# facebookresearch/Pearl

Hardware: NVIDIA H100
Metric: learner gradient-steps/sec (batch=256, 1e6 replay) (higher is better)
Workload: dtype f32 (3xTF32 tensor-core products, fp32 accumulate)

## Files before the change

### pearl_b200/csrc/dqn_tc.cu

```cuda
#include <math.h>
#include <stdarg.h>
#include <stdlib.h>

#include <new>

#include "dqn_common.cuh"
#include "sampler.cuh"
#include "umma.cuh"

using namespace prl;

int prl_sampler_params(const prl_buf *b, int k, prl::SamplerParams *sp, size_t *smem_bytes);

namespace {

constexpr int NTH = 256;
constexpr int HID = 64;
constexpr int MAX_B = 256;
constexpr int REG1 = 0, REG2 = 65536, REG3 = 131072, MISC_OFF = 196608;
constexpr int HALF = 32768;
constexpr int SBUF = 16384;
constexpr int TL = 144;
constexpr int AR_A_HI = 0, AR_A_LO = 18432, AR_E = 36864, AR_B_LO = 46080, AR_B_HI = REG3 + HALF;
constexpr int ACH = 1024, ARING = 8, ASLOT = 4 * ACH * 4;

struct TcLearner {
    const uint32_t *records;
    float *tiles;
    const int32_t *slots;
    float *w, *wt, *m, *v, *vmax;
    const float2 *scal;
    float *out_mae, *out_q, *out_y;
    long long steps0;
    int buf_flags;
    int pad_;
};

struct TcArgs {
    const TcLearner *learners;
    prl_buf_layout lay;
    Dims d;
    int B, rounds, freq;
    int round0;
    float decay, omb1, beta2, omb2, eps, gamma, tau, omtau, inv_b2;
    long long *prof;
    int prof_cta;
    int adam_tma;
};

__device__ __forceinline__ void tc_stamp(const TcArgs &a, int round, int idx) {
    long long *p = a.prof + (size_t)round * 16 + idx;
    const unsigned on = (a.prof != nullptr) & (blockIdx.x == (unsigned)a.prof_cta) & (threadIdx.x == 0);
    asm volatile("{\n\t.reg .pred q;\n\t.reg .u64 c;\n\tsetp.ne.u32 q, %1, 0;\n\tmov.u64 c, %%clock64;\n\t@q st.global.u64 [%0], c;\n\t}"
                 ::"l"(p), "r"(on) : "memory");
}
#define TC_STAMP(idx) tc_stamp(a, round, (idx))

struct Misc {
    struct Smalls { float watb[16][HID]; float b2[HID], w3[HID]; float b3, pad0[3]; } sm[2];
    float y[MAX_B];
    int act[MAX_B], cnt[MAX_B], slot[MAX_B];
    float rew[MAX_B], term[MAX_B];
    float redw[8][HID];
    float redmae[8], reddb3[8];
    unsigned long long bar[2 + ARING];
    TcLearner L;
    float dw3[16][NTH];
};

__device__ __forceinline__ void cp_async16_zfill_tc(void *smem_dst, const void *gmem_src, int src_bytes) {
    unsigned sa = (unsigned)__cvta_generic_to_shared(smem_dst);
    asm volatile("cp.async.cg.shared.global [%0], [%1], 16, %2;\n" ::"r"(sa), "l"(gmem_src), "r"(src_bytes) : "memory");
}

__device__ __forceinline__ int tid_here() {
    int t = threadIdx.x;
    asm volatile("" : "+r"(t));
    return t;
}
__device__ __forceinline__ int acc_row_here(int p) {
    const int t = tid_here();
    return ((t >> 5) & 3) * 16 + ((t & 31) >> 2) + 8 * p;
}
__device__ __forceinline__ void group_sync(int g) { asm volatile("bar.sync %0, %1;" ::"r"(1 + g), "r"(128) : "memory"); }

__device__ __forceinline__ void mbar_expect_tx(uint64_t *bar, uint32_t bytes) {
    asm volatile("mbarrier.arrive.expect_tx.shared::cta.b64 _, [%0], %1;" ::"r"(umma::smem_u32(bar)), "r"(bytes) : "memory");
}
__device__ __forceinline__ void bulk_g2s(void *smem_dst, const void *gmem_src, uint32_t bytes, uint64_t *bar) {
    asm volatile("cp.async.bulk.shared::cluster.global.mbarrier::complete_tx::bytes [%0], [%1], %2, [%3];"
                 ::"r"(umma::smem_u32(smem_dst)), "l"(gmem_src), "r"(bytes), "r"(umma::smem_u32(bar))
                 : "memory");
}
__device__ __forceinline__ void fence_proxy_async_all() { asm volatile("fence.proxy.async;" ::: "memory"); }
using umma::tf32_lo;

struct NetTiles { float *w1hi, *w1lo, *w2, *w2t; };
__host__ __device__ inline int k1_cols(int obs) { return (obs + 63) & ~63; }
__host__ __device__ inline int net_tile_floats(int obs) { return 128 * k1_cols(obs) + 2 * HID * HID; }
__device__ __forceinline__ NetTiles net_tiles(float *base, int obs, bool with_w2t) {
    const int k1 = k1_cols(obs), n = net_tile_floats(obs);
    return NetTiles{base, base + 64 * k1, base + 128 * k1, with_w2t ? base + n : nullptr};
}
__device__ void rebuild_tiles(const float *__restrict__ net, const Dims &d, const NetTiles &t, int tid) {
    const int k1 = k1_cols(d.obs);
    for (int e = tid; e < HID * k1; e += NTH) {
        const int j = e / k1, k = e - j * k1;
        const float x = k < d.obs ? __ldcg(net + d.oW1 + (size_t)j * d.D + k) : 0.f;
        const int idx = umma::tile_index(j, k, k1);
        t.w1hi[idx] = x; t.w1lo[idx] = tf32_lo(x);
    }
    for (int e = tid; e < HID * HID; e += NTH) {
        const int j = e >> 6, k = e & 63;
        const float x = __ldcg(net + d.oW2 + e);
        const int i1 = umma::tile_index(j, umma::kperm(k), HID);
        t.w2[i1] = x; t.w2[4096 + i1] = tf32_lo(x);
        if (t.w2t) {
            const int i2 = umma::tile_index(k, umma::kperm(j), HID);
            t.w2t[i2] = x; t.w2t[4096 + i2] = tf32_lo(x);
        }
    }
}
__device__ void load_smalls(const float *__restrict__ net, const Dims &d, Misc::Smalls &mi) {
    const int tid = tid_here();
    float wa[4], bb[4];
#pragma unroll
    for (int u = 0; u < 4; u++) {
        const int e = tid + u * NTH;
        if (e < d.A * HID) {
            const int j = e / d.A, a = e - j * d.A;
            wa[u] = __ldcg(net + d.oW1 + (size_t)j * d.D + d.obs + a);
            bb[u] = __ldcg(net + d.ob1 + j);
        }
    }
#pragma unroll
    for (int u = 0; u < 4; u++) {
        const int e = tid + u * NTH;
        if (e < d.A * HID) { const int j = e / d.A, a = e - j * d.A; mi.watb[a][j] = wa[u] + bb[u]; }
    }
    if (tid < HID) { mi.b2[tid] = __ldcg(net + d.ob2 + tid); mi.w3[tid] = __ldcg(net + d.oW3 + tid); }
    if (tid == 0) mi.b3 = __ldcg(net + d.ob3);
}

__device__ __forceinline__ float fast_sqrt(float x) {
    float r;
    asm("sqrt.approx.f32 %0, %1;" : "=f"(r) : "f"(x));
    return r;
}
struct AdamScalarsTc : AdamScalars { float inv_bc2_sqrt; };

__device__ __forceinline__ float adam_math(float w, float &m, float &v, float &x, float g, const AdamScalarsTc &hs) {
    float p = __fmul_rn(w, hs.decay);
    m = fmaf(hs.omb1, g - m, m);
    v = __fadd_rn(__fmul_rn(v, hs.beta2), __fmul_rn(__fmul_rn(hs.omb2, g), g));
    x = fmaxf(x, v);
    const float denom = __fadd_rn(__fmul_rn(fast_sqrt(x), hs.inv_bc2_sqrt), hs.eps);
    return __fadd_rn(p, __fdividef(__fmul_rn(-hs.step_size, m), denom));
}

__device__ __forceinline__ void l1_issue(const TcArgs &a, const TcLearner &L, const Misc &mi, char *smem, int field_off, int row0, int kc) {
    const int ft = tid_here(), m = ft & 127, g = ft >> 7;
    float *sbuf = reinterpret_cast<float *>(smem + REG2 + g * 2 * SBUF + (kc & 1) * SBUF);
#pragma unroll 4
    for (int i = 0; i < 8; i++) {
        const int item = i * 128 + m, rr = item >> 4, c = item & 15, k = kc * 64 + c * 4;
        const float *src = reinterpret_cast<const float *>(L.records + (size_t)mi.slot[row0 + rr] * a.lay.record_words) + field_off + k;
        const int nb = k < a.d.obs ? 16 : 0;
        cp_async16_zfill_tc(sbuf + rr * 64 + ((c ^ (rr & 7)) << 2), nb ? src : reinterpret_cast<const float *>(L.records), nb);
    }
    cp_async_commit();
}
__device__ __forceinline__ void layer1_block(const TcArgs &a, const TcLearner &L, const Misc &mi, char *smem, int field_off, int row0,
                                             float (&t1)[32]) {
    const int g = threadIdx.x >> 7;
    const int k1 = k1_cols(a.d.obs);
    const umma::Tile B_hi = umma::make_tile(smem + REG1, k1, 128), B_lo = umma::make_tile(smem + REG1 + HALF, k1, 128);
    for (int kc = 0; kc * 64 < k1; kc++) {
        if ((kc + 1) * 64 < k1) l1_issue(a, L, mi, smem, field_off, row0, kc + 1);
        else cp_async_commit();
        cp_async_wait<1>();
        group_sync(g);
        const float *sbuf = reinterpret_cast<const float *>(smem + REG2 + g * 2 * SBUF + (kc & 1) * SBUF);
        const int t = tid_here() & 3, r0 = acc_row_here(0);
        float hi[32], lo[32];
#pragma unroll
        for (int ks = 0; ks < 8; ks++)
#pragma unroll
            for (int q = 0; q < 2; q++)
#pragma unroll
                for (int p = 0; p < 2; p++) {
                    const int r = r0 + 8 * p, k = 8 * ks + t + 4 * q;
                    umma::split_tf32(sbuf[r * 64 + (((k >> 2) ^ (r & 7)) << 2) + (k & 3)], hi[4 * ks + 2 * q + p], lo[4 * ks + 2 * q + p]);
                }
        group_sync(g);
        umma::gemm3_rs<HID, 8>(t1, hi, lo, B_hi.shifted(kc * 2048), B_lo.shifted(kc * 2048), kc > 0);
        umma::wg_commit();
        umma::wg_wait<0>();
    }
}

__device__ __forceinline__ void acc_to_frag(const float (&v)[32], float (&hi)[32], float (&lo)[32]) {
#pragma unroll
    for (int j = 0; j < 8; j++)
#pragma unroll
        for (int p = 0; p < 2; p++)
#pragma unroll
            for (int e = 0; e < 2; e++) umma::split_tf32(v[4 * j + 2 * p + e], hi[4 * j + 2 * e + p], lo[4 * j + 2 * e + p]);
}

__device__ __forceinline__ float2 lds2(const float *p) {
    float2 v;
    asm volatile("ld.shared.v2.f32 {%0, %1}, [%2];" : "=f"(v.x), "=f"(v.y) : "r"(umma::smem_u32(p)));
    return v;
}

__device__ __forceinline__ float warp_sum(float v) {
#pragma unroll
    for (int o = 16; o; o >>= 1) v += __shfl_xor_sync(0xffffffffu, v, o);
    return v;
}
__device__ __forceinline__ float quad_sum(float v) {
    v += __shfl_xor_sync(0xffffffffu, v, 1);
    return v + __shfl_xor_sync(0xffffffffu, v, 2);
}

__host__ __device__ inline int dw1_share(int obs) { return obs > 64 ? 64 : obs > 32 ? 32 : obs > 16 ? 16 : 8; }

__device__ const uint8_t kIota[16] = {0, 1, 2, 3, 4, 5, 6, 7, 8, 9, 10, 11, 12, 13, 14, 15};

template <int NW>
__global__ void __launch_bounds__(NTH, 1) k_dqn_tc(const TcArgs a) {
    extern __shared__ __align__(1024) char smem[];
    Misc &mi = *reinterpret_cast<Misc *>(smem + MISC_OFF);
    const int tid = threadIdx.x, warp = tid >> 5, lane = tid & 31;
    if (tid == 0) {
        TcLearner L = a.learners[blockIdx.x];
        if (a.round0) {
            L.slots += (size_t)a.round0 * a.B;
            L.scal += a.round0;
            L.out_mae += a.round0;
            if (L.out_q) L.out_q += (size_t)a.round0 * a.B;
            if (L.out_y) L.out_y += (size_t)a.round0 * a.B;
            L.steps0 += a.round0;
        }
        mi.L = L;
    }
    __syncthreads();
    const TcLearner &L = mi.L;
    const Dims &d = a.d;
    const int h = tid >> 7, t4 = tid & 3;
    const int ntiles = a.B >> 7;
    const int W = a.lay.record_words;

    if (tid == 0 && gridDim.x > 1) {
        const long long t0 = clock64(), wait = (long long)(blockIdx.x % 48) * 2000;
        while (clock64() - t0 < wait) __nanosleep(100);
    }
    uint64_t *bar = reinterpret_cast<uint64_t *>(mi.bar);
    if (tid == 0)
        for (int i = 0; i < 2 + ARING; i++) umma::mbar_init(bar + i, 1);
    auto To = [&] { return net_tiles(L.tiles, d.obs, true); };
    auto Tt = [&] { return net_tiles(L.tiles + net_tile_floats(d.obs) + 2 * HID * HID, d.obs, false); };
    rebuild_tiles(L.w, d, To(), tid);
    rebuild_tiles(L.wt, d, Tt(), tid);
    fence_proxy_async_all();
    __syncthreads();
    const int k1 = k1_cols(d.obs);
    const uint32_t w1_bytes = 64u * k1 * 4, w2_bytes = 2u * HID * HID * 4;
    auto tma_online = [&](const NetTiles &t, uint64_t *b) {
        mbar_expect_tx(b, 2 * w1_bytes + 2 * w2_bytes);
        bulk_g2s(smem + REG1, t.w1hi, w1_bytes, b);
        bulk_g2s(smem + REG1 + HALF, t.w1lo, w1_bytes, b);
        bulk_g2s(smem + REG3, t.w2, 2 * w2_bytes, b);
    };
    const int an = d.ob2, nch = (an + ACH - 1) / ACH;
    auto aslot = [&](int s) { return smem + (s < 4 ? REG3 : REG1) + (s & 3) * ASLOT; };
    auto adam_issue = [&](int k) {
        const int off = k * ACH, s = k % ARING;
        const uint32_t bytes = 4u * (an - off < ACH ? an - off : ACH);
        char *dst = aslot(s);
        mbar_expect_tx(bar + 2 + s, 4 * bytes);
        bulk_g2s(dst, L.w + off, bytes, bar + 2 + s);
        bulk_g2s(dst + ACH * 4, L.m + off, bytes, bar + 2 + s);
        bulk_g2s(dst + ACH * 8, L.v + off, bytes, bar + 2 + s);
        bulk_g2s(dst + ACH * 12, L.vmax + off, bytes, bar + 2 + s);
    };
    uint32_t par_w1 = 0;
    const umma::Tile W2_hi = umma::make_tile(smem + REG3, 64, 128), W2_lo = umma::make_tile(smem + REG3 + 16384, 64, 128);
    const umma::Tile W2T_hi = umma::make_tile(smem + REG3 + 32768, 64, 128), W2T_lo = umma::make_tile(smem + REG3 + 49152, 64, 128);

    for (int round = 0; round < a.rounds; round++) {
        TC_STAMP(0);
        if (tid < a.B) {
            const int slot = L.slots[(size_t)round * a.B + tid];
            const uint32_t *r = L.records + (size_t)slot * W;
            mi.slot[tid] = slot;
            mi.act[tid] = (int)r[a.lay.off_action];
            mi.rew[tid] = __uint_as_float(r[a.lay.off_reward]);
            const uint32_t fl = r[a.lay.off_flags];
            mi.term[tid] = (fl & 1u) ? 1.f : 0.f;
            mi.cnt[tid] = (int)((fl >> 8) & 0xffffu);
            if (round + 1 < a.rounds) {
                const char *nx = reinterpret_cast<const char *>(L.records + (size_t)L.slots[(size_t)(round + 1) * a.B + tid] * W);
                for (int o = 0; o < W * 4; o += 128) asm volatile("prefetch.global.L2 [%0];" ::"l"(nx + o));
            }
        }
        const bool soft_upd = (L.steps0 + round + 2) % a.freq == 0;
        if (soft_upd) {
            for (int i = tid; i < d.P; i += NTH) L.wt[i] = soft_update(__ldcg(L.w + i), __ldcg(L.wt + i), a.tau, a.omtau);
            auto update_tile = [&](const float *on_hi, float *tg_hi, float *tg_lo, int n) {
                for (int i = tid * 4; i < n; i += NTH * 4) {
                    const float4 w = __ldcg(reinterpret_cast<const float4 *>(on_hi + i)), t = __ldcg(reinterpret_cast<const float4 *>(tg_hi + i));
                    const float4 r = make_float4(soft_update(w.x, t.x, a.tau, a.omtau), soft_update(w.y, t.y, a.tau, a.omtau),
                                                 soft_update(w.z, t.z, a.tau, a.omtau), soft_update(w.w, t.w, a.tau, a.omtau));
                    *reinterpret_cast<float4 *>(tg_hi + i) = r;
                    *reinterpret_cast<float4 *>(tg_lo + i) = make_float4(tf32_lo(r.x), tf32_lo(r.y), tf32_lo(r.z), tf32_lo(r.w));
                }
            };
            update_tile(To().w1hi, Tt().w1hi, Tt().w1lo, HID * k1);
            update_tile(To().w2, Tt().w2, Tt().w2 + HID * HID, HID * HID);
            fence_proxy_async_all();
        }
        __syncthreads();

        TC_STAMP(1);
        if (tid == 0) {
            mbar_expect_tx(bar + 0, 2 * w1_bytes + w2_bytes);
            bulk_g2s(smem + REG1, Tt().w1hi, w1_bytes, bar + 0);
            bulk_g2s(smem + REG1 + HALF, Tt().w1lo, w1_bytes, bar + 0);
            bulk_g2s(smem + REG3, Tt().w2, w2_bytes, bar + 0);
        }
        l1_issue(a, L, mi, smem, a.lay.off_next_state, h * 64, 0);
        if (soft_upd || round == 0) load_smalls(L.wt, d, mi.sm[1]);
        umma::mbar_wait(bar + 0, round & 1);
        __syncthreads();
        TC_STAMP(2);
        for (int i = 0; i < ntiles; i++) {
            const int row0 = i * 128 + h * 64;
            float t1[32];
            layer1_block(a, L, mi, smem, a.lay.off_next_state, row0, t1);
            if (i + 1 < ntiles) l1_issue(a, L, mi, smem, a.lay.off_next_state, row0 + 128, 0);
            else l1_issue(a, L, mi, smem, a.lay.off_state, h * 64, 0);
            const int rows[2] = {row0 + acc_row_here(0), row0 + acc_row_here(1)};
            int cnt[2];
            const uint8_t *ids[2];
            float best[2] = {-INFINITY, -INFINITY};
#pragma unroll
            for (int p = 0; p < 2; p++) {
                cnt[p] = mi.cnt[rows[p]];
                ids[p] = (L.buf_flags & PRL_BUF_DYNAMIC_ACTIONS) ? reinterpret_cast<const uint8_t *>(L.records + (size_t)mi.slot[rows[p]] * W + a.lay.off_avail)
                                                                : kIota;
            }
            for (int act = 0; act < d.A; act++) {
                const int t4 = tid_here() & 3;
                float hi[32], lo[32], acc[32];
#pragma unroll
                for (int p = 0; p < 2; p++) {
                    const int id_l = ids[p][act], id = act < cnt[p] ? id_l : act;
#pragma unroll
                    for (int j = 0; j < 8; j++) {
                        const float2 wv = lds2(&mi.sm[1].watb[id][8 * j + 2 * t4]);
                        umma::split_tf32(fmaxf(t1[4 * j + 2 * p] + wv.x, 0.f), hi[4 * j + p], lo[4 * j + p]);
                        umma::split_tf32(fmaxf(t1[4 * j + 2 * p + 1] + wv.y, 0.f), hi[4 * j + 2 + p], lo[4 * j + 2 + p]);
                    }
                }
                umma::gemm3_rs<HID, 8>(acc, hi, lo, W2_hi, W2_lo, false);
                umma::wg_commit();
                umma::wg_wait<0>();
                float q[2] = {0.f, 0.f};
#pragma unroll
                for (int j = 0; j < 8; j++) {
                    const float2 w3v = lds2(&mi.sm[1].w3[8 * j + 2 * t4]);
                    const float2 b2v = lds2(&mi.sm[1].b2[8 * j + 2 * t4]);
#pragma unroll
                    for (int p = 0; p < 2; p++) {
                        q[p] = fmaf(w3v.x, fmaxf(acc[4 * j + 2 * p] + b2v.x, 0.f), q[p]);
                        q[p] = fmaf(w3v.y, fmaxf(acc[4 * j + 2 * p + 1] + b2v.y, 0.f), q[p]);
                    }
                }
#pragma unroll
                for (int p = 0; p < 2; p++) {
                    float v = quad_sum(q[p]) + mi.sm[1].b3;
                    if (act >= cnt[p]) v = -INFINITY;
                    best[p] = fmaxf(best[p], v);
                }
            }
            if (t4 == 0)
#pragma unroll
                for (int p = 0; p < 2; p++)
                    mi.y[rows[p]] = __fadd_rn(__fmul_rn(__fmul_rn(best[p], a.gamma), 1.f - mi.term[rows[p]]), mi.rew[rows[p]]);
        }
        __syncthreads();

        TC_STAMP(3);
        if (tid == 0) tma_online(To(), bar + 1);
        load_smalls(L.w, d, mi.sm[0]);
        TC_STAMP(4);
        float gw2[16], gb2[4], gw1[NW / 2], gba[8];
        float mae_acc = 0.f, db3_acc = 0.f;
        float *arena = reinterpret_cast<float *>(smem);
        const umma::Tile TA_hi = umma::make_tile(smem + AR_A_HI, 64, TL), TA_lo = umma::make_tile(smem + AR_A_LO, 64, TL);
        const umma::Tile TB_hi = umma::make_tile(smem + AR_B_HI, 64, TL), TB_lo = umma::make_tile(smem + AR_B_LO, 64, TL);
        const umma::Tile TE = umma::make_tile(smem + AR_E, 64, TL);
        auto e_scatter = [&](int b0, int rA, int rB, int t4) {
#pragma unroll
            for (int p = 0; p < 2; p++) {
                const int r = p ? rB : rA, act = mi.act[b0 + r];
#pragma unroll
                for (int x = 0; x < 8; x++) {
                    const int er = t4 * 8 + x;
                    arena[AR_E / 4 + umma::tile_index2(er, r, 64, TL)] = (er == 0 || er == act + 1) ? 1.f : 0.f;
                }
            }
        };
        for (int i = 0; i < ntiles; i++) {
            const int row0 = i * 128 + h * 64;
            if (i > 0) {
                if (tid == 0) tma_online(To(), bar + 1);
                l1_issue(a, L, mi, smem, a.lay.off_state, row0, 0);
            }
            umma::mbar_wait(bar + 1, par_w1);
            par_w1 ^= 1;
            __syncthreads();
            const int rows[2] = {row0 + acc_row_here(0), row0 + acc_row_here(1)};
            float h1[32], z[32], hi[32], lo[32];
            layer1_block(a, L, mi, smem, a.lay.off_state, row0, h1);
            __syncthreads();
            if (i == 0) TC_STAMP(5);
            int ai[2];
#pragma unroll
            for (int p = 0; p < 2; p++) {
                ai[p] = mi.act[rows[p]];
#pragma unroll
                for (int j = 0; j < 8; j++) {
                    const float2 wv = lds2(&mi.sm[0].watb[ai[p]][8 * j + 2 * t4]);
                    h1[4 * j + 2 * p] = fmaxf(h1[4 * j + 2 * p] + wv.x, 0.f);
                    h1[4 * j + 2 * p + 1] = fmaxf(h1[4 * j + 2 * p + 1] + wv.y, 0.f);
                }
            }
            float *h1s = reinterpret_cast<float *>(smem + REG1 + h * HALF) + (tid & 127);
#pragma unroll
            for (int c = 0; c < 32; c++) h1s[c * 128] = h1[c];
            acc_to_frag(h1, hi, lo);
            umma::gemm3_rs<HID, 8>(z, hi, lo, W2_hi, W2_lo, false);
            umma::wg_commit();
            umma::wg_wait<0>();
            float part[2] = {0.f, 0.f}, dq[2];
#pragma unroll
            for (int j = 0; j < 8; j++) {
                const float2 w3v = lds2(&mi.sm[0].w3[8 * j + 2 * t4]);
                const float2 b2v = lds2(&mi.sm[0].b2[8 * j + 2 * t4]);
#pragma unroll
                for (int p = 0; p < 2; p++) {
                    z[4 * j + 2 * p] = fmaxf(z[4 * j + 2 * p] + b2v.x, 0.f);
                    z[4 * j + 2 * p + 1] = fmaxf(z[4 * j + 2 * p + 1] + b2v.y, 0.f);
                    part[p] = fmaf(w3v.x, z[4 * j + 2 * p], part[p]);
                    part[p] = fmaf(w3v.y, z[4 * j + 2 * p + 1], part[p]);
                }
            }
#pragma unroll
            for (int p = 0; p < 2; p++) {
                const float q = quad_sum(part[p]) + mi.sm[0].b3;
                const float y = mi.y[rows[p]];
                dq[p] = (q - y) * a.inv_b2;
                if (t4 == 0) {
                    if (L.out_q) L.out_q[(size_t)round * a.B + rows[p]] = q;
                    if (L.out_y) L.out_y[(size_t)round * a.B + rows[p]] = y;
                    mae_acc += fabsf(q - y);
                    db3_acc += dq[p];
                }
            }
#pragma unroll
            for (int j = 0; j < 8; j++) {
                const float2 w3v = lds2(&mi.sm[0].w3[8 * j + 2 * t4]);
                mi.dw3[2 * j][tid] = (i == 0 ? 0.f : mi.dw3[2 * j][tid]) + (dq[0] * z[4 * j] + dq[1] * z[4 * j + 2]);
                mi.dw3[2 * j + 1][tid] = (i == 0 ? 0.f : mi.dw3[2 * j + 1][tid]) + (dq[0] * z[4 * j + 1] + dq[1] * z[4 * j + 3]);
#pragma unroll
                for (int p = 0; p < 2; p++) {
                    z[4 * j + 2 * p] = z[4 * j + 2 * p] > 0.f ? dq[p] * w3v.x : 0.f;
                    z[4 * j + 2 * p + 1] = z[4 * j + 2 * p + 1] > 0.f ? dq[p] * w3v.y : 0.f;
                }
            }
            float dz1[32];
#pragma unroll
            for (int c = 0; c < 32; c++) h1s[(32 + c) * 128] = z[c];
            acc_to_frag(z, hi, lo);
            umma::gemm3_rs<HID, 8>(dz1, hi, lo, W2T_hi, W2T_lo, false);
            umma::wg_commit();
            umma::wg_wait<0>();
#pragma unroll
            for (int c = 0; c < 32; c++) {
                h1[c] = h1s[c * 128];
                z[c] = h1s[(32 + c) * 128];
                dz1[c] = (h1[c] > 0.f) ? dz1[c] : 0.f;
            }
            __syncthreads();
            float *dzs = reinterpret_cast<float *>(smem + REG3 + h * (HALF / 2)) + (tid & 127);
#pragma unroll
            for (int c = 0; c < 32; c++) dzs[c * 128] = dz1[c];
            if (i == 0) TC_STAMP(6);

            for (int hf = 0; hf < 2; hf++) {
                const int ft = tid_here(), h = ft >> 7, t4 = ft & 3, lane = ft & 31, warp = ft >> 5, rA = acc_row_here(0), rB = rA + 8;
                const bool mine = h == hf;
                const bool first = (i == 0 && hf == 0);
                __syncthreads();
                if (mine) {
#pragma unroll
                    for (int j = 0; j < 8; j++)
#pragma unroll
                        for (int p = 0; p < 2; p++)
#pragma unroll
                            for (int e = 0; e < 2; e++) {
                                const int idx = umma::tile_index2(8 * j + 2 * t4 + e, p ? rB : rA, 64, TL), c = 4 * j + 2 * p + e;
                                arena[AR_A_HI / 4 + idx] = z[c]; arena[AR_A_LO / 4 + idx] = tf32_lo(z[c]);
                                arena[AR_B_HI / 4 + idx] = h1[c]; arena[AR_B_LO / 4 + idx] = tf32_lo(h1[c]);
                            }
                } else {
                    e_scatter(i * 128 + hf * 64, rA, rB, t4);
                }
                umma::fence_async_smem();
                __syncthreads();
                if (first) TC_STAMP(11);
                umma::gemm3<32>(gw2, TA_hi, TA_lo, TB_hi.rows_from(32 * h), TB_lo.rows_from(32 * h), 64, !first);
                umma::gemm3<8>(gb2, TA_hi, TA_lo, TE, TE, 64, !first, false, true);
                umma::wg_commit();
                if (NW < 64 && lane < 16 && 32 * (lane & 3) < d.obs) {
                    const float *src = reinterpret_cast<const float *>(L.records + (size_t)mi.slot[i * 128 + hf * 64 + warp + 8 * (lane >> 2)] * W) +
                                       a.lay.off_state + 32 * (lane & 3);
                    asm volatile("prefetch.global.L1 [%0];" ::"l"(src));
                }
                umma::wg_wait<0>();
                if (first) TC_STAMP(12);
            }
            for (int hf = 0; hf < 2; hf++) {
                const int ft = tid_here(), h = ft >> 7, t4 = ft & 3, lane = ft & 31, warp = ft >> 5, rA = acc_row_here(0), rB = rA + 8;
                const bool mine = h == hf;
                const bool first = (i == 0 && hf == 0);
                __syncthreads();
                float sv[4][4];
                auto st_rows_load = [&](int r0) {
#pragma unroll
                    for (int ri = 0; ri < 4; ri++) {
                        const int rq = warp + 8 * (r0 + ri);
                        const float *src = reinterpret_cast<const float *>(L.records + (size_t)mi.slot[i * 128 + hf * 64 + rq] * W) + a.lay.off_state;
#pragma unroll
                        for (int jj = 0; jj < 4; jj++) sv[ri][jj] = (lane + 32 * jj < d.obs) ? __ldg(src + lane + 32 * jj) : 0.f;
                    }
                };
                auto st_rows_scatter = [&](int r0) {
#pragma unroll
                    for (int ri = 0; ri < 4; ri++) {
                        const int rq = warp + 8 * (r0 + ri);
#pragma unroll
                        for (int jj = 0; jj < 4; jj++)
                            if (lane + 32 * jj < d.obs) {
                                const int idx = umma::tile_index2(lane + 32 * jj, rq, 64, TL);
                                arena[AR_B_HI / 4 + idx] = sv[ri][jj]; arena[AR_B_LO / 4 + idx] = tf32_lo(sv[ri][jj]);
                            }
                    }
                };
                if constexpr (NW < 64) st_rows_load(0);
                if (mine) {
#pragma unroll
                    for (int j = 0; j < 8; j++)
#pragma unroll
                        for (int p = 0; p < 2; p++)
#pragma unroll
                            for (int e = 0; e < 2; e++) {
                                const int idx = umma::tile_index2(8 * j + 2 * t4 + e, p ? rB : rA, 64, TL), c = 4 * j + 2 * p + e;
                                const float v = reinterpret_cast<const float *>(smem + REG3 + h * (HALF / 2))[c * 128 + (ft & 127)];
                                arena[AR_A_HI / 4 + idx] = v; arena[AR_A_LO / 4 + idx] = tf32_lo(v);
                            }
                } else {
                    e_scatter(i * 128 + hf * 64, rA, rB, t4);
                }
                if constexpr (NW < 64) {
                    st_rows_scatter(0);
                    st_rows_load(4);
                    st_rows_scatter(4);
                }
                umma::fence_async_smem();
                __syncthreads();
                if (first) TC_STAMP(13);
                if constexpr (NW == 64) {
                    const float *sbuf = reinterpret_cast<const float *>(smem + REG2 + hf * 2 * SBUF + h * SBUF);
                    float shi[32], slo[32];
#pragma unroll
                    for (int ks = 0; ks < 8; ks++)
#pragma unroll
                        for (int q = 0; q < 2; q++)
#pragma unroll
                            for (int p = 0; p < 2; p++) {
                                const int o = p ? rB : rA, r = 8 * ks + t4 + 4 * q;
                                umma::split_tf32(sbuf[r * 64 + (((o >> 2) ^ (r & 7)) << 2) + (o & 3)], shi[4 * ks + 2 * q + p], slo[4 * ks + 2 * q + p]);
                            }
                    umma::gemm3_rs<64, 8, true>(gw1, shi, slo, TA_hi, TA_lo, !first);
                } else {
                    umma::gemm3<NW>(gw1, TA_hi, TA_lo, TB_hi.rows_from(NW * h), TB_lo.rows_from(NW * h), 64, !first);
                }
                umma::gemm3<16>(gba, TA_hi, TA_lo, TE.rows_from(16 * h), TE.rows_from(16 * h), 64, !first, false, true);
                umma::wg_commit();
                umma::wg_wait<0>();
                if (first) TC_STAMP(14);
            }
            umma::fence_async_smem();
            __syncthreads();
        }
        if (a.adam_tma && tid == 0)
            for (int k = 0; k < ARING && k < nch; k++) adam_issue(k);

        TC_STAMP(8);
#pragma unroll
        for (int c = 0; c < 16; c++) {
            float v = mi.dw3[c][tid];
            v += __shfl_xor_sync(0xffffffffu, v, 4);
            v += __shfl_xor_sync(0xffffffffu, v, 8);
            v += __shfl_xor_sync(0xffffffffu, v, 16);
            if (lane < 4) mi.redw[warp][8 * (c >> 1) + 2 * lane + (c & 1)] = v;
        }
        {
            const float ms = warp_sum(mae_acc), ds = warp_sum(db3_acc);
            if (lane == 0) { mi.redmae[warp] = ms; mi.reddb3[warp] = ds; }
        }
        {
            float *gs_w2 = reinterpret_cast<float *>(smem + REG2);
            const int pitch1 = d.D | 1;
            float *gs_w1 = gs_w2 + 64 * 65;
            float *gs_b1 = gs_w1 + 64 * pitch1, *gs_b2 = gs_b1 + 64;
#pragma unroll
            for (int p = 0; p < 2; p++) {
                const int j = acc_row_here(p);
#pragma unroll
                for (int jb = 0; jb < 4; jb++)
#pragma unroll
                    for (int e = 0; e < 2; e++) {
                        const int c = 8 * jb + 2 * t4 + e, x = 4 * jb + 2 * p + e;
                        gs_w2[j * 65 + 32 * h + c] = gw2[x];
                        if (NW < 64 && jb < NW / 8 && NW * h + c < d.obs) gs_w1[j * pitch1 + NW * h + c] = gw1[x];
                        if (jb < 2) {
                            const int ce = 16 * h + c;
                            if (ce == 0) gs_b1[j] = gba[x];
                            else if (ce - 1 < d.A) gs_w1[j * pitch1 + d.obs + ce - 1] = gba[x];
                        }
                    }
                if constexpr (NW == 64) {
                    const int k = 64 * h + j;
#pragma unroll
                    for (int jb = 0; jb < 8; jb++)
#pragma unroll
                        for (int e = 0; e < 2; e++)
                            if (k < d.obs) gs_w1[(8 * jb + 2 * t4 + e) * pitch1 + k] = gw1[4 * jb + 2 * p + e];
                }
                if (h == 0 && t4 == 0) gs_b2[j] = gb2[2 * p];
            }
            __syncthreads();
            TC_STAMP(7);
            const float2 sc = L.scal[round];
            AdamScalarsTc hs;
            hs.decay = a.decay; hs.omb1 = a.omb1; hs.beta2 = a.beta2; hs.omb2 = a.omb2; hs.eps = a.eps;
            hs.step_size = sc.x; hs.bc2_sqrt = sc.y; hs.inv_bc2_sqrt = 1.0f / sc.y;
            int si = -1;
            float sg = 0.f, sw = 0.f, sm = 0.f, sv2 = 0.f, sx = 0.f;
            if (tid < 64) { si = d.ob1 + tid; sg = gs_b1[tid]; }
            else if (tid < 128) { si = d.ob2 + tid - 64; sg = gs_b2[tid - 64]; }
            else if (tid < 192) {
                const int col = tid - 128;
                sg = 0.f;
#pragma unroll
                for (int w8 = 0; w8 < 8; w8++) sg += mi.redw[w8][col];
                si = d.oW3 + col;
            } else if (tid == 192) {
                float e = 0.f;
#pragma unroll
                for (int w8 = 0; w8 < 8; w8++) { sg += mi.reddb3[w8]; e += mi.redmae[w8]; }
                si = d.ob3;
                L.out_mae[round] = e / (float)a.B;
            }
            if (si >= 0) { sw = __ldcg(L.w + si); sm = __ldcg(L.m + si); sv2 = __ldcg(L.v + si); sx = __ldcg(L.vmax + si); }
            if (a.adam_tma) {
                const int n1 = HID * d.D;
                for (int k = 0; k < nch; k++) {
                    const int s = k % ARING, uses = (nch - 1 - s) / ARING + 1;
                    umma::mbar_wait(bar + 2 + s, (uint32_t)(round * uses + k / ARING) & 1u);
                    const int i = k * ACH + 4 * tid;
                    if (i < an && (i < n1 || i >= d.oW2)) {
                        const float4 *sl = reinterpret_cast<const float4 *>(aslot(s)) + tid;
                        float4 w = sl[0], mm = sl[ACH / 4], vv = sl[ACH / 2], xx = sl[3 * ACH / 4];
                        const bool is_w1 = i < n1;
                        int row, c;
                        const float *gp;
                        if (is_w1) {
                            row = i / d.D; c = i - row * d.D;
                            gp = gs_w1 + row * pitch1 + c;
                        } else {
                            const int e = i - d.oW2;
                            row = e >> 6; c = e & 63;
                            gp = gs_w2 + row * 65 + c;
                        }
                        w.x = adam_math(w.x, mm.x, vv.x, xx.x, gp[0], hs); w.y = adam_math(w.y, mm.y, vv.y, xx.y, gp[1], hs);
                        w.z = adam_math(w.z, mm.z, vv.z, xx.z, gp[2], hs); w.w = adam_math(w.w, mm.w, vv.w, xx.w, gp[3], hs);
                        *reinterpret_cast<float4 *>(L.w + i) = w; *reinterpret_cast<float4 *>(L.m + i) = mm;
                        *reinterpret_cast<float4 *>(L.v + i) = vv; *reinterpret_cast<float4 *>(L.vmax + i) = xx;
                        if (is_w1) {
                            if (c < d.obs) {
                                const int ti = umma::tile_index(row, c, k1);
                                *reinterpret_cast<float4 *>(To().w1hi + ti) = w;
                                *reinterpret_cast<float4 *>(To().w1lo + ti) = make_float4(tf32_lo(w.x), tf32_lo(w.y), tf32_lo(w.z), tf32_lo(w.w));
                            }
                        } else {
                            const int te = umma::tile_index(row, umma::kperm(c), HID), to = umma::tile_index(row, umma::kperm(c + 1), HID);
                            *reinterpret_cast<float2 *>(To().w2 + te) = make_float2(w.x, w.z);
                            *reinterpret_cast<float2 *>(To().w2 + to) = make_float2(w.y, w.w);
                            *reinterpret_cast<float2 *>(To().w2 + 4096 + te) = make_float2(tf32_lo(w.x), tf32_lo(w.z));
                            *reinterpret_cast<float2 *>(To().w2 + 4096 + to) = make_float2(tf32_lo(w.y), tf32_lo(w.w));
                            float *w2t = To().w2t;
                            const int kr = umma::kperm(row);
                            const float wv[4] = {w.x, w.y, w.z, w.w};
#pragma unroll
                            for (int u = 0; u < 4; u++) {
                                const int ti = umma::tile_index(c + u, kr, HID);
                                w2t[ti] = wv[u]; w2t[4096 + ti] = tf32_lo(wv[u]);
                            }
                        }
                    }
                    if (k + ARING < nch) {
                        __syncthreads();
                        if (tid == 0) adam_issue(k + ARING);
                    }
                }
            } else {
                for (int row = warp; row < HID; row += 8)
                    for (int c = lane; c < d.D; c += 32) {
                        const int i = d.oW1 + row * d.D + c;
                        float mm = __ldcg(L.m + i), vv = __ldcg(L.v + i), xx = __ldcg(L.vmax + i);
                        L.w[i] = adam_math(__ldcg(L.w + i), mm, vv, xx, gs_w1[row * pitch1 + c], hs);
                        L.m[i] = mm; L.v[i] = vv; L.vmax[i] = xx;
                    }
                for (int e = tid; e < HID * HID; e += NTH) {
                    const int i = d.oW2 + e;
                    float mm = __ldcg(L.m + i), vv = __ldcg(L.v + i), xx = __ldcg(L.vmax + i);
                    L.w[i] = adam_math(__ldcg(L.w + i), mm, vv, xx, gs_w2[(e >> 6) * 65 + (e & 63)], hs);
                    L.m[i] = mm; L.v[i] = vv; L.vmax[i] = xx;
                }
                __syncthreads();
                rebuild_tiles(L.w, d, To(), tid);
            }
            TC_STAMP(10);
            fence_proxy_async_all();
            if (si >= 0) {
                L.w[si] = adam_math(sw, sm, sv2, sx, sg, hs);
                L.m[si] = sm; L.v[si] = sv2; L.vmax[si] = sx;
            }
        }
        __syncthreads();
        TC_STAMP(9);
    }
}

__global__ void k_delay(unsigned ns) {
    const long long t0 = clock64();
    while (clock64() - t0 < (long long)ns * 2) __nanosleep(200);
}

struct MultiSampler {
    uint32_t *mt_state;
    SamplerParams sp;
};
__global__ void __launch_bounds__(kSamplerThreads, 1) k_sample_indices_multi(const MultiSampler *items, int rounds, int round0) {
    extern __shared__ __align__(16) unsigned char dyn[];
    __shared__ SamplerState S;
    MultiSampler it = items[blockIdx.x];
    if (it.sp.out_slot) it.sp.out_slot += (size_t)round0 * it.sp.k;
    if (it.sp.out_logical) it.sp.out_logical += (size_t)round0 * it.sp.k;
    sampler_init(S, it.mt_state, dyn, it.sp);
    sampler_advance(S, dyn, it.sp, rounds);
    __syncthreads();
    sampler_store(S, it.mt_state);
}

}

static bool tc_eligible(const prl_dqn_cfg &c, int batch) {
    const bool a_ok = c.n_actions == 1 || c.n_actions == 2 || c.n_actions == 4 || c.n_actions == 8 || c.n_actions == 16;
    return c.hidden1 == HID && c.hidden2 == HID && c.obs_dim % 8 == 0 && c.obs_dim >= 8 && c.obs_dim <= 128 && a_ok &&
           !c.double_dqn && (batch == 128 || batch == 256);
}

extern "C" int prl_dqn_tc_supported(const prl_dqn *q, int batch) { return q && q->tc_tiles && tc_eligible(q->cfg, batch) ? 1 : 0; }

extern "C" int prl_dqn_learn_multi(prl_dqn *const *dqns, prl_buf *const *bufs, int count, int rounds, int batch,
                                   const int64_t *training_steps0, float *const *out_mae, float *const *out_q,
                                   float *const *out_y, int32_t *const *out_logical, void *stream_) {
    PRL_REQUIRE(dqns && bufs && training_steps0 && out_mae && count > 0, "null / empty argument");
    cudaStream_t stream = (cudaStream_t)stream_;
    prl_dqn *q0 = dqns[0];
    const prl_dqn_cfg &c = q0->cfg;
    if (!tc_eligible(c, batch))
        return fail(PRL_EUNSUPPORTED,
                    "tensor-core learner needs hidden [64,64], obs %% 8 == 0 <= 128, actions in {1,2,4,8,16}, DQN, batch 128/256");
    PRL_REQUIRE(rounds > 0 && rounds <= c.max_rounds && batch <= c.max_batch, "rounds / batch outside the configured maxima");
    PRL_REQUIRE((size_t)count * (sizeof(TcLearner) + sizeof(MultiSampler)) <= 64 * 1024, "too many learners in one group");
    PRL_REQUIRE(count <= q0->sm_count, "more learners than SMs in one launch");
    static thread_local TcLearner *h_learn = nullptr;
    static thread_local MultiSampler *h_samp = nullptr;
    static thread_local cudaEvent_t h_done = nullptr;
    if (!h_learn) {
        PRL_CUDA(cudaHostAlloc((void **)&h_learn, 32 * 1024, cudaHostAllocDefault));
        PRL_CUDA(cudaHostAlloc((void **)&h_samp, 32 * 1024, cudaHostAllocDefault));
        PRL_CUDA(cudaEventCreateWithFlags(&h_done, cudaEventDisableTiming));
    }
    PRL_CUDA(cudaEventSynchronize(h_done));
    size_t samp_smem = 0;
    bool adam_tma = ((c.obs_dim + c.n_actions) & 3) == 0;
    for (int i = 0; i < count; i++) {
        prl_dqn *q = dqns[i];
        prl_buf *b = bufs[i];
        PRL_REQUIRE(q && b, "null learner / buffer");
        PRL_REQUIRE(b->shard_world <= 1, "buffer %d is one shard of a multi-GPU buffer: the tensor-core learner samples local buffers only", i);
        const prl_dqn_cfg &ci = q->cfg;
        PRL_REQUIRE(ci.obs_dim == c.obs_dim && ci.n_actions == c.n_actions && ci.hidden1 == c.hidden1 &&
                        ci.hidden2 == c.hidden2 && ci.double_dqn == c.double_dqn &&
                        ci.target_update_freq == c.target_update_freq && ci.lr == c.lr && ci.beta1 == c.beta1 &&
                        ci.beta2 == c.beta2 && ci.eps == c.eps && ci.weight_decay == c.weight_decay &&
                        ci.gamma == c.gamma && ci.tau == c.tau && rounds <= ci.max_rounds && batch <= ci.max_batch,
                    "all learners of a group must share one configuration");
        PRL_REQUIRE(q->tc_tiles, "learner %d has no operand-tile workspace", i);
        PRL_REQUIRE((b->desc.flags & PRL_BUF_DISCRETE) && b->desc.obs_dim == c.obs_dim && b->desc.n_actions == c.n_actions,
                    "buffer %d does not match the learner", i);
        PRL_REQUIRE(b->lay.record_words == bufs[0]->lay.record_words && b->lay.off_avail == bufs[0]->lay.off_avail,
                    "buffers must share one record layout");
        const bool shared_scal = i > 0 && q->adam_step == q0->adam_step;
        int rc = shared_scal ? PRL_OK : prl_dqn_stage_scalars(q, rounds, stream);
        if (rc) return rc;
        size_t sbytes = 0;
        rc = prl_sampler_params(b, batch, &h_samp[i].sp, &sbytes);
        if (rc) return rc;
        if (sbytes > samp_smem) samp_smem = sbytes;
        h_samp[i].mt_state = b->mt_state;
        h_samp[i].sp.out_slot = q->slots;
        h_samp[i].sp.out_logical = out_logical ? out_logical[i] : nullptr;
        TcLearner &L = h_learn[i];
        L.records = b->records; L.slots = q->slots;
        L.tiles = q->tc_tiles;
        L.w = q->w; L.wt = q->wt; L.m = q->m; L.v = q->v; L.vmax = q->vmax;
        adam_tma = adam_tma && (((uintptr_t)q->w | (uintptr_t)q->m | (uintptr_t)q->v | (uintptr_t)q->vmax) & 15) == 0;
        L.scal = shared_scal ? q0->scal_dev : q->scal_dev;
        L.out_mae = out_mae[i]; L.out_q = out_q ? out_q[i] : nullptr; L.out_y = out_y ? out_y[i] : nullptr;
        L.steps0 = training_steps0[i];
        L.buf_flags = b->desc.flags;
        L.pad_ = 0;
    }
    TcLearner *d_learn = reinterpret_cast<TcLearner *>(q0->multi_dev);
    MultiSampler *d_samp = reinterpret_cast<MultiSampler *>(reinterpret_cast<char *>(q0->multi_dev) + 32 * 1024);
    PRL_CUDA(cudaMemcpyAsync(d_learn, h_learn, (size_t)count * sizeof(TcLearner), cudaMemcpyHostToDevice, stream));
    PRL_CUDA(cudaMemcpyAsync(d_samp, h_samp, (size_t)count * sizeof(MultiSampler), cudaMemcpyHostToDevice, stream));
    PRL_CUDA(cudaEventRecord(h_done, stream));

    PRL_CUDA(cudaFuncSetAttribute(k_sample_indices_multi, cudaFuncAttributeMaxDynamicSharedMemorySize, 200 * 1024));

    TcArgs a;
    a.learners = d_learn;
    a.lay = bufs[0]->lay;
    a.d = q0->d;
    a.B = batch; a.rounds = rounds; a.freq = c.target_update_freq; a.round0 = 0;
    a.decay = (float)(1.0 - c.lr * c.weight_decay);
    a.omb1 = (float)(1.0 - c.beta1);
    a.beta2 = (float)c.beta2;
    a.omb2 = (float)(1.0 - c.beta2);
    a.eps = (float)c.eps;
    a.gamma = (float)c.gamma;
    a.tau = (float)c.tau;
    a.omtau = (float)(1.0 - c.tau);
    a.inv_b2 = 2.0f / (float)batch;
    a.adam_tma = adam_tma ? 1 : 0;
    a.prof = q0->prof;
    { static const int c = [] { const char *e = getenv("PRL_TC_PROF_CTA"); return e ? atoi(e) : 0; }(); a.prof_cta = c; }
    const size_t smem = MISC_OFF + sizeof(Misc);
    PRL_REQUIRE(smem <= (size_t)q0->max_smem, "tensor-core learner needs %zu B of shared memory", smem);
    const int nw = dw1_share(c.obs_dim);
    void (*const kern)(TcArgs) = nw == 64 ? k_dqn_tc<64> : nw == 32 ? k_dqn_tc<32> : nw == 16 ? k_dqn_tc<16> : k_dqn_tc<8>;
    PRL_CUDA(cudaFuncSetAttribute(kern, cudaFuncAttributeMaxDynamicSharedMemorySize, (int)smem));

    const int spare = q0->sm_count - count;
    int nchunks = 1;
    if (!q0->prof && spare >= 2 && rounds >= 64) nchunks = rounds >= 256 ? 4 : 2;
    static thread_local cudaStream_t side = nullptr;
    static thread_local cudaEvent_t ev_idx[8], ev_fork = nullptr;
    if (nchunks > 1 && !side) {
        PRL_CUDA(cudaStreamCreateWithFlags(&side, cudaStreamNonBlocking));
        for (auto &e : ev_idx) PRL_CUDA(cudaEventCreateWithFlags(&e, cudaEventDisableTiming));
        PRL_CUDA(cudaEventCreateWithFlags(&ev_fork, cudaEventDisableTiming));
    }
    const int first = nchunks > 1 ? (rounds / nchunks < 32 ? rounds / nchunks : 32) : rounds;
    auto chunk_begin = [&](int cix) {
        return cix == 0 ? 0 : first + (int)((long long)(rounds - first) * (cix - 1) / (nchunks > 1 ? nchunks - 1 : 1));
    };
    k_sample_indices_multi<<<count, kSamplerThreads, samp_smem, stream>>>(d_samp, chunk_begin(1), 0);
    PRL_CUDA(cudaGetLastError());
    if (nchunks > 1) {
        PRL_CUDA(cudaEventRecord(ev_fork, stream));
        PRL_CUDA(cudaStreamWaitEvent(side, ev_fork, 0));
    }
    if (q0->timing) PRL_CUDA(cudaEventRecord(q0->t0, stream));
    for (int cix = 0; cix < nchunks; cix++) {
        const int r0 = chunk_begin(cix), r1 = chunk_begin(cix + 1);
        if (cix > 0) PRL_CUDA(cudaStreamWaitEvent(stream, ev_idx[cix], 0));
        a.round0 = r0; a.rounds = r1 - r0;
        kern<<<count, NTH, smem, stream>>>(a);
        PRL_CUDA(cudaGetLastError());
        if (cix + 1 < nchunks) {
            const int n0 = r1, n1 = chunk_begin(cix + 2);
            k_delay<<<1, 1, 0, side>>>(30000u);
            k_sample_indices_multi<<<count, kSamplerThreads, samp_smem, side>>>(d_samp, n1 - n0, n0);
            PRL_CUDA(cudaGetLastError());
            PRL_CUDA(cudaEventRecord(ev_idx[cix + 1], side));
        }
    }
    if (q0->timing) PRL_CUDA(cudaEventRecord(q0->t1, stream));
    for (int i = 0; i < count; i++) {
        dqns[i]->adam_step += rounds;
        dqns[i]->last_launches = 3 * nchunks - 1;
        dqns[i]->last_ctas = 1;
        dqns[i]->last_rows = batch;
    }
    return PRL_OK;
}
```

Baseline: 545,100.

## Alternate warpgroup GEMM issue with turn barriers and spill action tables to smem

Adds named-barrier turn passing so the two 128-thread warpgroups take turns issuing the per-action target-network wgmma. One group's epilogue can then overlap the other's tensor-core work. Per-row action ids, masks and running maxima are precomputed into shared-memory tables instead of registers, which reduces register pressure in the action loop. The cost is extra barrier traffic, more shared-memory loads and stores, and an async-proxy fence before the block sync. It also risks deadlock if barrier counts mismatch.

```diff
diff --git a/pearl_b200/csrc/dqn_tc.cu b/pearl_b200/csrc/dqn_tc.cu
--- a/pearl_b200/csrc/dqn_tc.cu
+++ b/pearl_b200/csrc/dqn_tc.cu
@@ -83,6 +83,17 @@
     return ((t >> 5) & 3) * 16 + ((t & 31) >> 2) + 8 * p;
 }
 __device__ __forceinline__ void group_sync(int g) { asm volatile("bar.sync %0, %1;" ::"r"(1 + g), "r"(128) : "memory"); }
+
+__device__ __forceinline__ void turn_wait() { asm volatile("bar.sync %0, 256;" ::"r"(3 + (tid_here() >> 7)) : "memory"); }
+__device__ __forceinline__ void turn_pass() {
+    asm volatile("{\n\t.reg .pred q;\n\tsetp.lt.u32 q, %0, 128;\n\t@q bar.arrive 4, 256;\n\t@!q bar.arrive 3, 256;\n\t}" ::"r"(tid_here()) : "memory");
+}
+__device__ __forceinline__ void turn_open() {
+    asm volatile("{\n\t.reg .pred q;\n\tsetp.ne.u32 q, %0, 0;\n\t@q bar.arrive 3, 256;\n\t}" ::"r"(tid_here() >> 7) : "memory");
+}
+__device__ __forceinline__ void turn_close() {
+    asm volatile("{\n\t.reg .pred q;\n\tsetp.eq.u32 q, %0, 0;\n\t@q bar.sync 3, 256;\n\t}" ::"r"(tid_here() >> 7) : "memory");
+}
 
 __device__ __forceinline__ void mbar_expect_tx(uint64_t *bar, uint32_t bytes) {
     asm volatile("mbarrier.arrive.expect_tx.shared::cta.b64 _, [%0], %1;" ::"r"(umma::smem_u32(bar)), "r"(bytes) : "memory");
@@ -289,6 +300,7 @@
     const umma::Tile W2_hi = umma::make_tile(smem + REG3, 64, 128), W2_lo = umma::make_tile(smem + REG3 + 16384, 64, 128);
     const umma::Tile W2T_hi = umma::make_tile(smem + REG3 + 32768, 64, 128), W2T_lo = umma::make_tile(smem + REG3 + 49152, 64, 128);
 
+    turn_open();
     for (int round = 0; round < a.rounds; round++) {
         TC_STAMP(0);
         if (tid < a.B) {
@@ -337,26 +349,36 @@
         TC_STAMP(2);
         for (int i = 0; i < ntiles; i++) {
             const int row0 = i * 128 + h * 64;
+#pragma unroll
+            for (int p = 0; p < 2; p++) {
+                const int cnt = mi.cnt[row0 + acc_row_here(p)];
+                const uint8_t *ids = (L.buf_flags & PRL_BUF_DYNAMIC_ACTIONS)
+                                         ? reinterpret_cast<const uint8_t *>(L.records + (size_t)mi.slot[row0 + acc_row_here(p)] * W + a.lay.off_avail)
+                                         : kIota;
+                uint8_t *tab = reinterpret_cast<uint8_t *>(smem + REG3 + HALF) + p * 16 * NTH + tid_here();
+#pragma unroll 4
+                for (int k = 0; k < 16; k++) {
+                    const int id = ids[k < d.A ? k : d.A - 1];
+                    tab[k * NTH] = (uint8_t)(k < cnt ? id : k | 0x80);
+                }
+            }
             float t1[32];
             layer1_block(a, L, mi, smem, a.lay.off_next_state, row0, t1);
             if (i + 1 < ntiles) l1_issue(a, L, mi, smem, a.lay.off_next_state, row0 + 128, 0);
             else l1_issue(a, L, mi, smem, a.lay.off_state, h * 64, 0);
             const int rows[2] = {row0 + acc_row_here(0), row0 + acc_row_here(1)};
-            int cnt[2];
-            const uint8_t *ids[2];
-            float best[2] = {-INFINITY, -INFINITY};
-#pragma unroll
-            for (int p = 0; p < 2; p++) {
-                cnt[p] = mi.cnt[rows[p]];
-                ids[p] = (L.buf_flags & PRL_BUF_DYNAMIC_ACTIONS) ? reinterpret_cast<const uint8_t *>(L.records + (size_t)mi.slot[rows[p]] * W + a.lay.off_avail)
-                                                                : kIota;
+            {
+                float *bests = reinterpret_cast<float *>(smem + REG3 + HALF + 2 * 16 * NTH) + tid_here();
+                bests[0] = -INFINITY;
+                bests[NTH] = -INFINITY;
             }
             for (int act = 0; act < d.A; act++) {
                 const int t4 = tid_here() & 3;
+                const uint8_t *tab = reinterpret_cast<const uint8_t *>(smem + REG3 + HALF) + act * NTH + tid_here();
                 float hi[32], lo[32], acc[32];
 #pragma unroll
                 for (int p = 0; p < 2; p++) {
-                    const int id_l = ids[p][act], id = act < cnt[p] ? id_l : act;
+                    const int id = tab[p * 16 * NTH] & 0x7f;
 #pragma unroll
                     for (int j = 0; j < 8; j++) {
                         const float2 wv = lds2(&mi.sm[1].watb[id][8 * j + 2 * t4]);
@@ -364,14 +386,18 @@
                         umma::split_tf32(fmaxf(t1[4 * j + 2 * p + 1] + wv.y, 0.f), hi[4 * j + 2 + p], lo[4 * j + 2 + p]);
                     }
                 }
+                turn_wait();
                 umma::gemm3_rs<HID, 8>(acc, hi, lo, W2_hi, W2_lo, false);
                 umma::wg_commit();
+                turn_pass();
                 umma::wg_wait<0>();
+                const int t4e = tid_here() & 3;
+                const uint8_t *tabe = reinterpret_cast<const uint8_t *>(smem + REG3 + HALF) + act * NTH + tid_here();
                 float q[2] = {0.f, 0.f};
 #pragma unroll
                 for (int j = 0; j < 8; j++) {
-                    const float2 w3v = lds2(&mi.sm[1].w3[8 * j + 2 * t4]);
-                    const float2 b2v = lds2(&mi.sm[1].b2[8 * j + 2 * t4]);
+                    const float2 w3v = lds2(&mi.sm[1].w3[8 * j + 2 * t4e]);
+                    const float2 b2v = lds2(&mi.sm[1].b2[8 * j + 2 * t4e]);
 #pragma unroll
                     for (int p = 0; p < 2; p++) {
                         q[p] = fmaf(w3v.x, fmaxf(acc[4 * j + 2 * p] + b2v.x, 0.f), q[p]);
@@ -381,15 +407,19 @@
 #pragma unroll
                 for (int p = 0; p < 2; p++) {
                     float v = quad_sum(q[p]) + mi.sm[1].b3;
-                    if (act >= cnt[p]) v = -INFINITY;
-                    best[p] = fmaxf(best[p], v);
-                }
-            }
+                    if (tabe[p * 16 * NTH] & 0x80) v = -INFINITY;
+                    float *bp = reinterpret_cast<float *>(smem + REG3 + HALF + 2 * 16 * NTH) + p * NTH + tid_here();
+                    *bp = fmaxf(*bp, v);
+                }
+            }
+            const float *bests = reinterpret_cast<const float *>(smem + REG3 + HALF + 2 * 16 * NTH) + tid_here();
+            const float best[2] = {bests[0], bests[NTH]};
             if (t4 == 0)
 #pragma unroll
                 for (int p = 0; p < 2; p++)
                     mi.y[rows[p]] = __fadd_rn(__fmul_rn(__fmul_rn(best[p], a.gamma), 1.f - mi.term[rows[p]]), mi.rew[rows[p]]);
         }
+        umma::fence_async_smem();
         __syncthreads();
 
         TC_STAMP(3);
@@ -756,6 +786,7 @@
         __syncthreads();
         TC_STAMP(9);
     }
+    turn_close();
 }
 
 __global__ void k_delay(unsigned ns) {
```

New measurement: 586,000 (median of 6 runs). 7.5% higher.
